# olsson-group/thermodynamic-interpolation

Measured on AMD Instinct MI355X. Metric: integration-steps/sec (whole node) + drift rel-L2 vs CPU ref, higher is better.
Workload: dtype f32 state and accumulation; matrix products on fp16 MFMA with 2-way split fp32 operands (hi + lo halves, 3 products)

## Files before the change

thermodynamic-interpolation_amd/csrc/painn_pair_kernel_body.inc:

```
{
    static_assert(PREC == 0 || PREC == 1, "the fp16 storage mode keeps the directed message kernel");
    constexpr int F = 16 * NBK, NB = (F + 31) / 32, T = 64 * WAVES, CH4 = edge_chunk4(NB, false);
    using A16 = r16::Act<NBK>;
    constexpr bool ONE = edge_one_chain(NB, PREC);
    using OP = std::conditional_t<ONE, r16::Opnd1<NBK>, typename r16::OpSel<NBK, PREC>::type>;
    extern __shared__ f32x4 lds[];
    const int lane = threadIdx.x & 63, wave = __builtin_amdgcn_readfirstlane(threadIdx.x >> 6), j = lane & 15, q = lane >> 4;
    constexpr int SC = pair_superchunk(), NBUF = pair_ring(WAVES);
    float* scratch = reinterpret_cast<float*>(lds + NBUF * SC * CH4) + wave * 64;
    float* vec = reinterpret_cast<float*>(lds + NBUF * SC * CH4) + WAVES * 64;
    for (int i = threadIdx.x; i < EV::COUNT * F / 4; i += T)
        reinterpret_cast<f32x4*>(vec)[i] = reinterpret_cast<const f32x4*>(p.vecs)[i];
#ifndef TI_PAIR_STAGGER
#define TI_PAIR_STAGGER 0
#endif
    PipeDMA<NB, T, SC, CH4, WAVES == 8 && TI_PAIR_STAGGER, NBUF> pipe;
    pipe.init(reinterpret_cast<const f32x4*>(p.stream), p.nch, lds, wave, lane);

    const float eps_w0 = ONE ? 1e-5f * p.wscale[0] * p.wscale[0] : 1e-5f, eps_w1 = ONE ? 1e-5f * p.wscale[1] * p.wscale[1] : 1e-5f;
    const float eps_p0 = ONE ? 1e-5f * p.wscale[2] * p.wscale[2] : 1e-5f, eps_p1 = ONE ? 1e-5f * p.wscale[3] * p.wscale[3] : 1e-5f;
    const float s_p0 = ONE ? p.wscale[2] : 1.0f, inv_out = ONE ? 1.0f / (p.wscale[4] * p.wscale[5]) : 1.0f;
    const long long gi_raw = (long long)blockIdx.x * WAVES + wave;
    const bool group_ok = gi_raw < p.n_groups;
    const long long gi = group_ok ? gi_raw : p.n_groups - 1;
    auto node_of = [&](int mol_local, int atom) {
        long long m = gi * p.G + mol_local;
        m = m < p.B ? m : p.B - 1;
        return m * p.A + atom;
    };

#ifdef TI_STAMPS
    constexpr int STAMP_SLOTS = 64;
    const bool st_wg = blockIdx.x >= 300 && blockIdx.x < 304;
    unsigned long long* const st_buf = p.stamps ? p.stamps + ((size_t)(blockIdx.x - 300) * WAVES + wave) * STAMP_SLOTS : nullptr;
    int st_i = 0;
    unsigned long long clk0 = 0, rt0 = 0;
    if (p.stamps) { clk0 = __builtin_amdgcn_s_memtime(); rt0 = __builtin_amdgcn_s_memrealtime(); }
#define TI_STAMP() do { if (st_wg && st_buf && blk == 3 && st_i < STAMP_SLOTS) { const unsigned long long t_ = __builtin_amdgcn_s_memtime(); if (lane == 0) st_buf[st_i] = t_; ++st_i; } } while (0)
#else
#define TI_STAMP() do { } while (0)
#endif

    for (int blk = 0; blk < p.nblk; ++blk) {
        TI_STAMP();
        const uint32_t meta = TI_PAIR_ROWS[blk * 16 + j];
        const long long nI = node_of(prow_molI(meta), prow_atomI(meta)), nJ = node_of(prow_molJ(meta), prow_atomJ(meta));
        const size_t brow0 = ((size_t)gi * p.nblk + blk) * 16;
        const size_t erowA = brow0 * 2, erowB = erowA + 16;
        OP enc;
        f32x4* const enc_park = reinterpret_cast<f32x4*>(p.enc) + (brow0 / 16) * (sizeof(OP) / 16) * 64 + lane;
        f32x4* const geo_park = reinterpret_cast<f32x4*>(p.geo) + brow0 + j;
        if constexpr (FIRST) {
            const float rx = p.x[nI * 3 + 0] - p.x[nJ * 3 + 0];
            const float ry = p.x[nI * 3 + 1] - p.x[nJ * 3 + 1];
            const float rz = p.x[nI * 3 + 2] - p.x[nJ * 3 + 2];
            const float dist = sqrtf(rx * rx + ry * ry + rz * rz);
            const float den = 1.0f + dist;
            if (q == 0) {
                f32x4 dd = {rx / den, ry / den, rz / den, 0.f};
                *reinterpret_cast<f32x4*>(scratch + j * 4) = dd;
                if (group_ok) *geo_park = dd;
            }
            A16 t;
            r16::posenc_set(t, dist / p.length_scale, q);
            enc.set(t);
            if (group_ok) r16::opnd_store(enc, enc_park);
        } else {
            if (q == 0) *reinterpret_cast<f32x4*>(scratch + j * 4) = *geo_park;
            r16::opnd_load(enc, enc_park);
        }
        TI_STAMP();
        OP g2;
        {
            OP g1;
            A16 t1;
#pragma unroll
            for (int c = 0; c < NB; ++c) {
                f32x4 a0 = r16::load_block(vec + EV::W_B0 * F, 2 * c, q), a1 = r16::load_block(vec + EV::W_B0 * F, 2 * c + 1, q);
                r16::gemm_on_pipe<false>(a0, a1, enc, pipe, lane);
                t1.b[2 * c] = a0; t1.b[2 * c + 1] = a1;
                pipe.release();
            }
            TI_STAMP();
            r16::ln_silu(t1, vec + EV::W_G0 * F, vec + EV::W_BE0 * F, q, eps_w0);
            g1.set(t1);
            TI_STAMP();
#pragma unroll
            for (int c = 0; c < NB; ++c) {
                f32x4 a0 = r16::load_block(vec + EV::W_B1 * F, 2 * c, q), a1 = r16::load_block(vec + EV::W_B1 * F, 2 * c + 1, q);
                r16::gemm_on_pipe<false>(a0, a1, g1, pipe, lane);
                t1.b[2 * c] = a0; t1.b[2 * c + 1] = a1;
                pipe.release();
            }
            TI_STAMP();
            r16::ln_silu(t1, vec + EV::W_G1 * F, vec + EV::W_BE1 * F, q, eps_w1);
            g2.set(t1);
            TI_STAMP();
        }
        OP h2A, h2B;
        {
            OP inA, inB;
            A16 tA, tB;
            float scA, scB;
            if (FIRST) {
                r16::load_set(tA, p.edge_emb + prow_type(meta) * F, q);
                scA = inA.set_scaled(tA);
                inB = inA; scB = scA;
            } else {
                r16::load_set(tA, p.e + (erowA + j) * F, q);
                r16::load_set(tB, p.e + (erowB + j) * F, q);
                scA = inA.set_scaled(tA);
                scB = inB.set_scaled(tB);
            }
            const float ivA = r16::pow2_inverse(scA) * s_p0, ivB = r16::pow2_inverse(scB) * s_p0;
            TI_STAMP();
#pragma unroll
            for (int c = 0; c < NB; ++c) {
                f32x4 a0 = r16::load_state<false>(p.P, (size_t)nI * F, 2 * c, q) * ivA, a1 = r16::load_state<false>(p.P, (size_t)nI * F, 2 * c + 1, q) * ivA;
                f32x4 b0 = r16::load_state<false>(p.P, (size_t)nJ * F, 2 * c, q) * ivB, b1 = r16::load_state<false>(p.P, (size_t)nJ * F, 2 * c + 1, q) * ivB;
                r16::gemm_x2_on_pipe<false>(a0, a1, b0, b1, inA, inB, pipe, lane);
                tA.b[2 * c] = a0 * scA; tA.b[2 * c + 1] = a1 * scA;
                tB.b[2 * c] = b0 * scB; tB.b[2 * c + 1] = b1 * scB;
                pipe.release();
            }
            TI_STAMP();
            r16::ln_silu(tA, vec + EV::P_G0 * F, vec + EV::P_BE0 * F, q, eps_p0);
            r16::ln_silu(tB, vec + EV::P_G0 * F, vec + EV::P_BE0 * F, q, eps_p0);
            inA.set(tA); inB.set(tB);
            TI_STAMP();
#pragma unroll
            for (int c = 0; c < NB; ++c) {
                f32x4 a0 = r16::load_block(vec + EV::P_B1 * F, 2 * c, q), a1 = r16::load_block(vec + EV::P_B1 * F, 2 * c + 1, q);
                f32x4 b0 = a0, b1 = a1;
                r16::gemm_x2_on_pipe<false>(a0, a1, b0, b1, inA, inB, pipe, lane);
                tA.b[2 * c] = a0; tA.b[2 * c + 1] = a1;
                tB.b[2 * c] = b0; tB.b[2 * c + 1] = b1;
                pipe.release();
            }
            TI_STAMP();
            r16::ln_silu(tA, vec + EV::P_G1 * F, vec + EV::P_BE1 * F, q, eps_p1);
            r16::ln_silu(tB, vec + EV::P_G1 * F, vec + EV::P_BE1 * F, q, eps_p1);
            h2A.set(tA); h2B.set(tB);
            TI_STAMP();
        }
        uint32_t mi[4];
#pragma unroll
        for (int r = 0; r < 4; ++r) mi[r] = TI_PAIR_ROWS[blk * 16 + 4 * q + r];
        f32x4 wfac;
#pragma unroll
        for (int r = 0; r < 4; ++r) wfac[r] = (mi[r] & 1u) ? inv_out : 0.0f;
#ifndef TI_PAIR_ACC_ATOMIC
#define TI_PAIR_ACC_ATOMIC 1
#endif
        float* const part_blk = p.part + ((size_t)gi * p.nblk + blk) * 8 * (7 * F);
        const int snJ = p.slotnode[blk * 16 + 4 + q], snI = p.slotnode[blk * 16 + q];
        const bool haveA = group_ok && snJ >= 0 && (!TI_PAIR_ACC_ATOMIC || gi * p.G + slot_mol(snJ) < p.B);
        const bool haveB = group_ok && snI >= 0 && (!TI_PAIR_ACC_ATOMIC || gi * p.G + slot_mol(snI) < p.B);
        float* const partA = part_blk + (size_t)(4 + q) * (7 * F);
        float* const partB = part_blk + (size_t)q * (7 * F);
        const int qnA = (int)((gi * p.G + slot_mol(snJ)) * p.A) + (snJ & 255), qnB = (int)((gi * p.G + slot_mol(snI)) * p.A) + (snI & 255);
        const bool qfA = (snJ & SLOT_FIRST_TOUCH) != 0, qfB = (snI & SLOT_FIRST_TOUCH) != 0;
        auto acc_ptr = [&](int node, int off) {
            return off < F ? p.dsacc + (size_t)node * F + off : off < 4 * F ? p.dvacc + (size_t)node * 3 * F + (off - F) : p.cacc + (size_t)node * 3 * F + (off - 4 * F);
        };
        const long long nIq = node_of(prow_molI(mi[0]), prow_atomI(mi[0]));

        auto out3 = [&](int c, int nbo, f32x4& rA0, f32x4& rA1, f32x4& rB0, f32x4& rB1) {
            f32x4 a0 = {0, 0, 0, 0}, a1 = {0, 0, 0, 0}, b0 = {0, 0, 0, 0}, b1 = {0, 0, 0, 0}, w0 = {0, 0, 0, 0}, w1 = {0, 0, 0, 0};
            r16::gemm_x2_on_pipe<true>(a0, a1, b0, b1, h2A, h2B, pipe, lane);
            pipe.release();
            r16::gemm_on_pipe<true>(w0, w1, g2, pipe, lane);
            pipe.release();
            const float* bp = vec + (EV::P_B2 + c) * F + 32 * nbo + j;
            const float* bw = vec + (EV::W_B2 + c) * F + 32 * nbo + j;
            w0 = (w0 + bw[0]) * wfac; w1 = (w1 + bw[16]) * wfac;
            rA0 = (a0 + bp[0]) * w0; rA1 = (a1 + bp[16]) * w1;
            rB0 = (b0 + bp[0]) * w0; rB1 = (b1 + bp[16]) * w1;
        };
        auto sumA = [&](const f32x4& v) {
            using QS = r16::QuarterSum<4>;
            return QS::swap32_add(QS::swap16_add(v[0], v[1]), QS::swap16_add(v[2], v[3]));
        };
        auto putA = [&](float z0, float z1, int off) {
            if (TI_PAIR_ACC_ATOMIC) { if (haveA) { float* d = acc_ptr(qnA, off); acc_out(d, z0, qfA); acc_out(d + 16, z1, qfA); } }
            else if (haveA) { partA[off] = z0; partA[off + 16] = z1; }
        };
        auto putB = [&](float z0, float z1, int off) {
            if (TI_PAIR_ACC_ATOMIC) { if (haveB) { float* d = acc_ptr(qnB, off); acc_out(d, z0, qfB); acc_out(d + 16, z1, qfB); } }
            else if (haveB) { partB[off] = z0; partB[off + 16] = z1; }
        };
        auto sumB = [&](const f32x4& v) { return (v[0] + v[1]) + (v[2] + v[3]); };
        auto emitA = [&](const f32x4& v0, const f32x4& v1, int off) { putA(sumA(v0), sumA(v1), off); };
        auto emitB = [&](const f32x4& v0, const f32x4& v1, int off) { putB(sumB(v0), sumB(v1), off); };
        auto rows4 = [&](float x, float (&o)[4]) {
            float a = x, b = x;
            lane_swap16(a, b);
            o[0] = a; o[2] = a; lane_swap32(o[0], o[2]);
            o[1] = b; o[3] = b; lane_swap32(o[1], o[3]);
        };
        constexpr bool GATHER_EARLY = PREC != 0;
        constexpr bool FOLD = pair_folds_cross(PREC) && !FIRST;
        f32x4* const zpark = reinterpret_cast<f32x4*>(vec + EV::COUNT * F) + wave * 3 * 64 + lane;
        static_assert(!FOLD || GATHER_EARLY, "the fold crosses with the v[dst] rows that the early gathers hold");
        const long long nJq = snJ >= 0 ? node_of(slot_mol(snJ), snJ & 255) : nIq;
        const float wrow = (meta & 1u) ? inv_out : 0.0f;

#pragma unroll 1
        for (int nbo = 0; nbo < NB; ++nbo) {
            const int fo = 32 * nbo + j;
            TI_STAMP();
            {
                f32x4 a0, a1, b0, b1;
                out3(2, nbo, a0, a1, b0, b1);
                emitA(a0, a1, fo);
                emitB(b0, b1, fo);
            }
            TI_STAMP();
            if constexpr (!LAST) {
                f32x4 a0 = r16::load_block(vec + (EV::P_B2 + 3) * F, 2 * nbo, q), a1 = r16::load_block(vec + (EV::P_B2 + 3) * F, 2 * nbo + 1, q);
                f32x4 b0 = a0, b1 = a1;
                f32x4 w0 = r16::load_block(vec + (EV::W_B2 + 3) * F, 2 * nbo, q), w1 = r16::load_block(vec + (EV::W_B2 + 3) * F, 2 * nbo + 1, q);
                float* const ea = p.e + (erowA + j) * F;
                float* const eb = p.e + (erowB + j) * F;
                f32x4 oA0, oA1, oB0, oB1;
                if (FIRST) {
                    const float* em = p.edge_emb + prow_type(meta) * F;
                    oA0 = r16::load_block(em, 2 * nbo, q); oA1 = r16::load_block(em, 2 * nbo + 1, q);
                    oB0 = oA0; oB1 = oA1;
                } else {
                    oA0 = r16::load_block(ea, 2 * nbo, q); oA1 = r16::load_block(ea, 2 * nbo + 1, q);
                    oB0 = r16::load_block(eb, 2 * nbo, q); oB1 = r16::load_block(eb, 2 * nbo + 1, q);
                }
                r16::gemm_x2_on_pipe<false>(a0, a1, b0, b1, h2A, h2B, pipe, lane);
                pipe.release();
                r16::gemm_on_pipe<false>(w0, w1, g2, pipe, lane);
                pipe.release();
                w0 *= wrow; w1 *= wrow;
                if (group_ok) {
                    r16::store_block(ea, 2 * nbo, q, oA0 + a0 * w0); r16::store_block(ea, 2 * nbo + 1, q, oA1 + a1 * w1);
                    r16::store_block(eb, 2 * nbo, q, oB0 + b0 * w0); r16::store_block(eb, 2 * nbo + 1, q, oB1 + b1 * w1);
                }
            }
            TI_STAMP();
            {
                f32x4 sA0, sA1, sB0, sB1, gA0 = {0, 0, 0, 0}, gA1 = {0, 0, 0, 0}, gB0 = {0, 0, 0, 0}, gB1 = {0, 0, 0, 0};
                out3(1, nbo, sA0, sA1, sB0, sB1);
                float vI[3][2], vJ[3][2];
                if (!FIRST) {
                    const float* vp = p.v + (size_t)nIq * 3 * F + fo;
                    const float* vq = p.v + (size_t)nJq * 3 * F + fo;
#pragma unroll
                    for (int c = 0; c < 3; ++c) {
                        vI[c][0] = vp[c * F]; vI[c][1] = vp[c * F + 16];
                        if (GATHER_EARLY) { vJ[c][0] = vq[c * F]; vJ[c][1] = vq[c * F + 16]; }
                    }
                    out3(0, nbo, gA0, gA1, gB0, gB1);
                }
                f32x4 dir[4];
#pragma unroll
                for (int r = 0; r < 4; ++r) dir[r] = *reinterpret_cast<const f32x4*>(scratch + (4 * q + r) * 4);
                float zA[3][2], zB[3][2];
#pragma unroll
                for (int c = 0; c < 3; ++c) {
                    f32x4 v0, v1;
#pragma unroll
                    for (int r = 0; r < 4; ++r) {
                        v0[r] = sA0[r] * dir[r][c]; v1[r] = sA1[r] * dir[r][c];
                        if (!FIRST) { v0[r] = fmaf(gA0[r], vI[c][0], v0[r]); v1[r] = fmaf(gA1[r], vI[c][1], v1[r]); }
                    }
                    zA[c][0] = sumA(v0); zA[c][1] = sumA(v1);
                    if (!GATHER_EARLY) putA(zA[c][0], zA[c][1], (1 + c) * F + fo);
                }
#pragma unroll
                for (int c = 0; c < 3; ++c) {
                    f32x4 v0, v1;
                    float j0[4], j1[4];
                    if (!FIRST) {
                        if (GATHER_EARLY) { rows4(vJ[c][0], j0); rows4(vJ[c][1], j1); }
                        else
#pragma unroll
                            for (int r = 0; r < 4; ++r) {
                                const float* vr = p.v + (size_t)node_of(prow_molJ(mi[r]), prow_atomJ(mi[r])) * 3 * F + c * F + fo;
                                j0[r] = vr[0]; j1[r] = vr[16];
                            }
                    }
#pragma unroll
                    for (int r = 0; r < 4; ++r) {
                        v0[r] = -(sB0[r] * dir[r][c]); v1[r] = -(sB1[r] * dir[r][c]);
                        if (!FIRST) { v0[r] = fmaf(gB0[r], j0[r], v0[r]); v1[r] = fmaf(gB1[r], j1[r], v1[r]); }
                    }
                    zB[c][0] = sumB(v0); zB[c][1] = sumB(v1);
                    if (!GATHER_EARLY) putB(zB[c][0], zB[c][1], (1 + c) * F + fo);
                }
                TI_STAMP();
                if constexpr (FOLD) {
                    zpark[0] = f32x4{zA[0][0], zA[0][1], zA[1][0], zA[1][1]};
                    zpark[64] = f32x4{zA[2][0], zA[2][1], zB[0][0], zB[0][1]};
                    zpark[128] = f32x4{zB[1][0], zB[1][1], zB[2][0], zB[2][1]};
                    f32x4 cA0, cA1, cB0, cB1;
                    out3(4, nbo, cA0, cA1, cB0, cB1);
                    f32x4 dc[4];
#pragma unroll
                    for (int r = 0; r < 4; ++r) dc[r] = *reinterpret_cast<const f32x4*>(scratch + (4 * q + r) * 4);
                    {
                        const f32x4 z0 = zpark[0], z1 = zpark[64], z2 = zpark[128];
                        zA[0][0] = z0[0]; zA[0][1] = z0[1]; zA[1][0] = z0[2]; zA[1][1] = z0[3];
                        zA[2][0] = z1[0]; zA[2][1] = z1[1]; zB[0][0] = z1[2]; zB[0][1] = z1[3];
                        zB[1][0] = z2[0]; zB[1][1] = z2[1]; zB[2][0] = z2[2]; zB[2][1] = z2[3];
                    }
                    float kA[3][2], kB[3][2];
#pragma unroll
                    for (int c = 0; c < 3; ++c) {
                        f32x4 a0, a1, b0, b1;
#pragma unroll
                        for (int r = 0; r < 4; ++r) {
                            a0[r] = cA0[r] * dc[r][c]; a1[r] = cA1[r] * dc[r][c];
                            b0[r] = -(cB0[r] * dc[r][c]); b1[r] = -(cB1[r] * dc[r][c]);
                        }
                        kA[c][0] = sumA(a0); kA[c][1] = sumA(a1);
                        kB[c][0] = sumB(b0); kB[c][1] = sumB(b1);
                    }
#pragma unroll
                    for (int c = 0; c < 3; ++c) {
                        const int c1 = (c + 1) % 3, c2 = (c + 2) % 3;
#pragma unroll
                        for (int h = 0; h < 2; ++h) {
                            zA[c][h] += kA[c1][h] * vJ[c2][h] - kA[c2][h] * vJ[c1][h];
                            zB[c][h] += kB[c1][h] * vI[c2][h] - kB[c2][h] * vI[c1][h];
                        }
                    }
                }
                if (GATHER_EARLY)
#pragma unroll
                    for (int c = 0; c < 3; ++c) { putA(zA[c][0], zA[c][1], (1 + c) * F + fo); putB(zB[c][0], zB[c][1], (1 + c) * F + fo); }
                if (!FIRST && !FOLD) {
                    f32x4 cA0, cA1, cB0, cB1;
                    out3(4, nbo, cA0, cA1, cB0, cB1);
#pragma unroll
                    for (int c = 0; c < 3; ++c) {
                        f32x4 v0, v1;
#pragma unroll
                        for (int r = 0; r < 4; ++r) { v0[r] = cA0[r] * dir[r][c]; v1[r] = cA1[r] * dir[r][c]; }
                        emitA(v0, v1, (4 + c) * F + fo);
                    }
#pragma unroll
                    for (int c = 0; c < 3; ++c) {
                        f32x4 v0, v1;
#pragma unroll
                        for (int r = 0; r < 4; ++r) { v0[r] = -(cB0[r] * dir[r][c]); v1[r] = -(cB1[r] * dir[r][c]); }
                        emitB(v0, v1, (4 + c) * F + fo);
                    }
                }
            }
        }
    }
    pipe.drain();
#ifdef TI_STAMPS
    if (p.stamps && lane == 0) {
        const unsigned long long clk1 = __builtin_amdgcn_s_memtime(), rt1 = __builtin_amdgcn_s_memrealtime();
        unsigned long long* c = p.stamps + 2048 + 2 * (size_t)gi_raw;
        c[0] = clk1 - clk0; c[1] = rt1 - rt0;
    }
#endif
}
```

thermodynamic-interpolation_amd/csrc/ti_api.hip:

```cpp
#include <algorithm>
#include <array>
#include <climits>
#include <cmath>
#include <cstdio>
#include <cstdlib>
#include <cstring>
#include <map>
#include <memory>
#include <stdexcept>
#include <utility>

#include "pair_template.hpp"
#include "ti_internal.hpp"

namespace ti {

static thread_local std::string g_err;
static int fail(int code, const std::string& msg) { g_err = msg; return code; }

struct HipError : std::runtime_error { using std::runtime_error::runtime_error; };
struct Unsupported : std::runtime_error { using std::runtime_error::runtime_error; };
#define HIP_CHECK(expr) do { hipError_t e__ = (expr); if (e__ != hipSuccess) \
    throw HipError(std::string(#expr) + ": " + hipGetErrorString(e__)); } while (0)

// ... 1617 lines not shown
        const float *xd = x, *cd = cond, *td = t; float *od = out, *dd = out_div;
        if (mem == TI_MEM_HOST) {
            if (h->rk_tv.n < (size_t)B) h->rk_tv.alloc(B);
            HIP_CHECK(hipMemcpyAsync(h->x.p, x, n * sizeof(float), hipMemcpyHostToDevice, h->stream));
            if (nc) HIP_CHECK(hipMemcpyAsync(h->cond.p, cond, nc * sizeof(float), hipMemcpyHostToDevice, h->stream));
            HIP_CHECK(hipMemcpyAsync(h->rk_tv.p, t, (size_t)B * sizeof(float), hipMemcpyHostToDevice, h->stream));
            xd = h->x.p; cd = h->cond.p; td = h->rk_tv.p; od = h->b1.p; dd = h->divb.p;
        }
        painn_drift_div_dev(h, xd, 0.f, cd, B, od, dd, td);
        if (mem == TI_MEM_HOST) {
            HIP_CHECK(hipMemcpyAsync(out, od, n * sizeof(float), hipMemcpyDeviceToHost, h->stream));
            HIP_CHECK(hipMemcpyAsync(out_div, dd, (size_t)B * sizeof(float), hipMemcpyDeviceToHost, h->stream));
        }
        HIP_CHECK(hipStreamSynchronize(h->stream));
        return TI_OK;
    });
}

static int painn_rollout_dlogp_impl(ti_handle* h, const ti_rollout_desc* rd, int n_probes, uint64_t probe_seed, const float* x0,
                                    const float* cond, int64_t B, float div_scale, float out_scale, int reverse_ode, float* out_path,
                                    float* out_dlogp, int64_t* n_fevals)
{
    if (!h || h->kind != 0) return fail(TI_E_ARG, "not a painn handle");
    if (h->d.precision == TI_PREC_F16) return fail(TI_E_UNSUPPORTED, "the fp16 storage mode has no divergence / tangent path (use f32 or f16x2)");
    if (int rc = check_rollout_desc(rd)) return rc;
    if (rd->scheme == TI_SCHEME_EM) return fail(TI_E_UNSUPPORTED, "dlogp is defined for the deterministic schemes only (EULER, HEUN)");
    if (rd->scheme == TI_SCHEME_DOPRI5_TRAJ && h->obs[1].K > 0)
        return fail(TI_E_UNSUPPORTED, "TI_SCHEME_DOPRI5_TRAJ writes its rows per trajectory inside a kernel: detach the observer (ti_obs_set_observer)");
    if (B < 0 || (B > 0 && (!x0 || !out_path || !out_dlogp || (h->ncond > 0 && !cond)))) return fail(TI_E_ARG, "NULL buffer");
    if (B == 0) { if (n_fevals) *n_fevals = 0; return TI_OK; }
    return guarded([&]() -> int {
        set_device(h);
        select_template(h, B, false);
        ensure_painn_ws(h, B);
        const int A = h->d.n_atoms;
        const size_t n = (size_t)B * A * 3, nc = (size_t)B * A * h->ncond;
        const hipMemcpyKind in_kind = rd->mem == TI_MEM_DEVICE ? hipMemcpyDeviceToDevice : hipMemcpyHostToDevice;
        HIP_CHECK(hipMemcpyAsync(h->x.p, x0, n * sizeof(float), in_kind, h->stream));
        const float* cd = cond;
        if (rd->mem == TI_MEM_HOST && nc) { HIP_CHECK(hipMemcpyAsync(h->cond.p, cond, nc * sizeof(float), hipMemcpyHostToDevice, h->stream)); cd = h->cond.p; }
        const int saved_tap = h->tap; h->tap = -1;
        const Ragged rg = ragged_of(h);
        if (n_probes > 0) painn_make_probes(h, B, n_probes, probe_seed, rd->traj_offset);
        DlogpAux aux;
        aux.dl = h->dl.p; aux.d1 = h->divb.p; aux.d2 = h->div2.p; aux.scaled = h->dlscaled.p; aux.out = out_dlogp;
        aux.n_dl = (size_t)B; aux.div_scale = div_scale; aux.out_scale = out_scale;
        auto drift = [&](const float* xs, float t, float* o, float* dv) {
            if (n_probes > 0) painn_drift_div_est_dev(h, xs, t, cd, B, n_probes, o, dv);
            else painn_drift_div_dev(h, xs, t, cd, B, o, dv);
            if (reverse_ode) {
                HIP_CHECK(launch_scale(o, o, -1.0f, (long long)n, h->stream));
                HIP_CHECK(launch_scale(dv, dv, -1.0f, (long long)B, h->stream));
            }
        };
        auto drift_tv = [&](const float* xs, const float* tv, float* o, float* dv) {
            if (n_probes > 0) painn_drift_div_est_dev(h, xs, 0.f, cd, B, n_probes, o, dv, tv);
            else painn_drift_div_dev(h, xs, 0.f, cd, B, o, dv, tv);
            if (reverse_ode) {
                HIP_CHECK(launch_scale(o, o, -1.0f, (long long)n, h->stream));
                HIP_CHECK(launch_scale(dv, dv, -1.0f, (long long)B, h->stream));
            }
        };
        const int rc = rd->scheme == TI_SCHEME_DOPRI5_TRAJ ? rollout_rk_traj(h, rd, h->x.p, B, A * 3, out_path, n_fevals, drift_tv, aux, rg)
                     : rd->scheme >= TI_SCHEME_DOPRI5 ? rollout_rk(h, rd, h->x.p, n, out_path, n_fevals, drift, aux, rg)
                                                      : rollout_common(h, rd, h->x.p, h->b1.p, h->b2.p, h->xt.p, n, B, A * 3, A, out_path, n_fevals, drift, aux, rg);
        h->tap = saved_tap;
        return rc;
    });
}

int ti_painn_rollout_dlogp(ti_handle* h, const ti_rollout_desc* rd, const float* x0, const float* cond, int64_t B, float div_scale,
                           float out_scale, int reverse_ode, float* out_path, float* out_dlogp, int64_t* n_fevals)
{
    return painn_rollout_dlogp_impl(h, rd, 0, 0, x0, cond, B, div_scale, out_scale, reverse_ode, out_path, out_dlogp, n_fevals);
}

int ti_painn_rollout_dlogp_est(ti_handle* h, const ti_rollout_desc* rd, int32_t n_probes, uint64_t probe_seed, const float* x0,
                               const float* cond, int64_t B, float div_scale, float out_scale, int reverse_ode, float* out_path,
                               float* out_dlogp, int64_t* n_fevals)
{
    if (!h || h->kind != 0) return fail(TI_E_ARG, "not a painn handle");
    if (h->d.precision == TI_PREC_F16) return fail(TI_E_UNSUPPORTED, "the fp16 storage mode has no divergence / tangent path (use f32 or f16x2)");
    if (n_probes < 1) return fail(TI_E_ARG, "n_probes must be >= 1");
    return painn_rollout_dlogp_impl(h, rd, n_probes, probe_seed, x0, cond, B, div_scale, out_scale, reverse_ode, out_path, out_dlogp, n_fevals);
}

static int painn_drift_div_est_impl(ti_handle* h, const float* x, float t, const float* tv, const float* cond, int64_t B, int32_t n_probes,
                                    uint64_t probe_seed, int64_t traj_offset, float* out, float* out_div, int mem, bool per_mol_t)
{
    if (!h || h->kind != 0) return fail(TI_E_ARG, "not a painn handle");
    if (h->d.precision == TI_PREC_F16) return fail(TI_E_UNSUPPORTED, "the fp16 storage mode has no divergence / tangent path (use f32 or f16x2)");
    if (n_probes < 1) return fail(TI_E_ARG, "n_probes must be >= 1");
    if (B < 0 || (B > 0 && (!x || (per_mol_t && !tv) || !out || !out_div || (h->ncond > 0 && !cond)))) return fail(TI_E_ARG, "NULL buffer");
    if (B == 0) return TI_OK;
    if (h->tap >= 0) return fail(TI_E_ARG, "debug taps apply to ti_painn_drift / ti_painn_drift_jvp only");
    return guarded([&]() -> int {
        set_device(h);
        select_template(h, B, false);
        ensure_painn_ws(h, B);
        const size_t n = (size_t)B * h->d.n_atoms * 3, nc = (size_t)B * h->d.n_atoms * h->ncond;
        const float *xd = x, *cd = cond, *td = tv; float *od = out, *dd = out_div;
        if (mem == TI_MEM_HOST) {
            HIP_CHECK(hipMemcpyAsync(h->x.p, x, n * sizeof(float), hipMemcpyHostToDevice, h->stream));
            if (nc) HIP_CHECK(hipMemcpyAsync(h->cond.p, cond, nc * sizeof(float), hipMemcpyHostToDevice, h->stream));
            if (per_mol_t) {
                if (h->rk_tv.n < (size_t)B) h->rk_tv.alloc(B);
                HIP_CHECK(hipMemcpyAsync(h->rk_tv.p, tv, (size_t)B * sizeof(float), hipMemcpyHostToDevice, h->stream));
                td = h->rk_tv.p;
            }
            xd = h->x.p; cd = h->cond.p; od = h->b1.p; dd = h->divb.p;
        }
        painn_make_probes(h, B, n_probes, probe_seed, traj_offset);
        painn_drift_div_est_dev(h, xd, t, cd, B, n_probes, od, dd, per_mol_t ? td : nullptr);
        if (mem == TI_MEM_HOST) {
            HIP_CHECK(hipMemcpyAsync(out, od, n * sizeof(float), hipMemcpyDeviceToHost, h->stream));
            HIP_CHECK(hipMemcpyAsync(out_div, dd, (size_t)B * sizeof(float), hipMemcpyDeviceToHost, h->stream));
        }
        HIP_CHECK(hipStreamSynchronize(h->stream));
        return TI_OK;
    });
}

int ti_painn_drift_div_est(ti_handle* h, const float* x, float t, const float* cond, int64_t B, int32_t n_probes, uint64_t probe_seed,
                           int64_t traj_offset, float* out, float* out_div, int mem)
{
    return painn_drift_div_est_impl(h, x, t, nullptr, cond, B, n_probes, probe_seed, traj_offset, out, out_div, mem, false);
}

int ti_painn_drift_div_est_tv(ti_handle* h, const float* x, const float* t, const float* cond, int64_t B, int32_t n_probes,
                              uint64_t probe_seed, int64_t traj_offset, float* out, float* out_div, int mem)
{
    return painn_drift_div_est_impl(h, x, 0.f, t, cond, B, n_probes, probe_seed, traj_offset, out, out_div, mem, true);
}

int ti_painn_debug_tap(ti_handle* h, int stage)
{
    if (!h || h->kind != 0) return fail(TI_E_ARG, "not a painn handle");
    if (h->d.precision == TI_PREC_F16 && stage >= 0) return fail(TI_E_UNSUPPORTED, "debug taps read fp32 state; not available in the fp16 storage mode");
    h->tap = stage;
    return TI_OK;
}

int ti_painn_debug_poison(ti_handle* h, int64_t B, float value)
{
    if (!h || h->kind != 0 || B <= 0) return fail(TI_E_ARG, "not a painn handle / B");
    return guarded([&]() -> int {
        set_device(h);
        ensure_painn_ws(h, B);
        const size_t N = (size_t)B * h->d.n_atoms, F = h->d.n_features;
        const unsigned bits = __builtin_bit_cast(unsigned, value);
        HIP_CHECK(hipMemsetD32Async((hipDeviceptr_t)h->dsacc.p, (int)bits, N * F, h->stream));
        HIP_CHECK(hipMemsetD32Async((hipDeviceptr_t)h->dvacc.p, (int)bits, N * 3 * F, h->stream));
        HIP_CHECK(hipMemsetD32Async((hipDeviceptr_t)h->cacc.p, (int)bits, N * 3 * F, h->stream));
        return TI_OK;
    });
}

int ti_painn_debug_read(ti_handle* h, int what, float* out, size_t n_floats)
{
    if (!h || h->kind != 0 || !out) return fail(TI_E_ARG, "bad argument");
    return guarded([&]() -> int {
        set_device(h);
        const size_t A = h->d.n_atoms, F = h->d.n_features, E = h->d.n_edges, B = (size_t)h->last_B, N = B * A;
        HIP_CHECK(hipStreamSynchronize(h->stream));
        if (what == 0) {
            if (n_floats != N * F) return fail(TI_E_ARG, "size mismatch (s)");
            std::vector<float> ds(n_floats);
            HIP_CHECK(hipMemcpy(out, h->s.p, n_floats * sizeof(float), hipMemcpyDeviceToHost));
            HIP_CHECK(hipMemcpy(ds.data(), h->dsacc.p, n_floats * sizeof(float), hipMemcpyDeviceToHost));
            for (size_t i = 0; i < n_floats; ++i) out[i] += ds[i];
        } else if (what == 1) {
            if (n_floats != N * 3 * F) return fail(TI_E_ARG, "size mismatch (v)");
            std::vector<float> v(n_floats), dv(n_floats), cc(n_floats);
            HIP_CHECK(hipMemcpy(v.data(), h->v.p, n_floats * sizeof(float), hipMemcpyDeviceToHost));
            HIP_CHECK(hipMemcpy(dv.data(), h->dvacc.p, n_floats * sizeof(float), hipMemcpyDeviceToHost));
            HIP_CHECK(hipMemcpy(cc.data(), h->cacc.p, n_floats * sizeof(float), hipMemcpyDeviceToHost));
            for (size_t nd = 0; nd < N; ++nd)
                for (size_t f = 0; f < F; ++f)
                    for (int c = 0; c < 3; ++c) {
                        const int c1 = (c + 1) % 3, c2 = (c + 2) % 3;
                        auto at = [&](const std::vector<float>& a, int cc2) { return a[(nd * 3 + cc2) * F + f]; };
                        out[(nd * 3 + c) * F + f] = (at(v, c) + at(dv, c)) + (at(cc, c1) * at(v, c2) - at(cc, c2) * at(v, c1));
                    }
        } else if (what == 2) {
            if (n_floats != B * E * F) return fail(TI_E_ARG, "size mismatch (e)");
            const size_t RB = ti::EDGE_ROWS_PER_BLOCK, rows = (B + h->G - 1) / h->G * h->parts * h->nblk * RB * (h->active == 2 ? 2 : 1);
            std::vector<float> e(rows * F);
            HIP_CHECK(hipMemcpy(e.data(), h->e.p, e.size() * sizeof(float), hipMemcpyDeviceToHost));
            for (size_t m = 0; m < B; ++m)
                for (size_t k = 0; k < E; ++k)
                    std::memcpy(out + (m * E + h->perm[k]) * F, e.data() + edge_row_of(h, m, k) * F, F * sizeof(float));
        } else if (what >= 3 && what <= 5) {
            if (h->last_D != 1 || (size_t)h->last_VB != B) return fail(TI_E_ARG, "tangent taps need a preceding ti_painn_drift_jvp call");
            auto fetch = [&](const DevBuf<float>& b, size_t n) { std::vector<float> v(n); HIP_CHECK(hipMemcpy(v.data(), b.p, n * sizeof(float), hipMemcpyDeviceToHost)); return v; };
            if (what == 3) {
                if (n_floats != N * F) return fail(TI_E_ARG, "size mismatch (ts)");
                const auto ts = fetch(h->ts, n_floats), td = fetch(h->tdsacc, n_floats);
                for (size_t i = 0; i < n_floats; ++i) out[i] = ts[i] + td[i];
            } else if (what == 4) {
                if (n_floats != N * 3 * F) return fail(TI_E_ARG, "size mismatch (tv)");
                const auto v = fetch(h->v, n_floats), cc = fetch(h->cacc, n_floats);
                const auto tv = fetch(h->tv, n_floats), tdv = fetch(h->tdvacc, n_floats), tcc = fetch(h->tcacc, n_floats);
                for (size_t nd = 0; nd < N; ++nd)
                    for (size_t f = 0; f < F; ++f)
                        for (int c = 0; c < 3; ++c) {
                            const int c1 = (c + 1) % 3, c2 = (c + 2) % 3;
                            auto at = [&](const std::vector<float>& a, int cc2) { return a[(nd * 3 + cc2) * F + f]; };
                            out[(nd * 3 + c) * F + f] = (at(tv, c) + at(tdv, c)) + ((at(tcc, c1) * at(v, c2) + at(cc, c1) * at(tv, c2)) -
                                                                                     (at(tcc, c2) * at(v, c1) + at(cc, c2) * at(tv, c1)));
                        }
            } else {
                if (n_floats != B * E * F) return fail(TI_E_ARG, "size mismatch (te)");
                const size_t RB = ti::EDGE_ROWS_PER_BLOCK, rows = (B + h->G - 1) / h->G * h->parts * h->nblk * RB;
                const auto e = fetch(h->te, rows * F);
                for (size_t m = 0; m < B; ++m)
                    for (size_t k = 0; k < E; ++k)
                        std::memcpy(out + (m * E + h->perm[k]) * F, e.data() + edge_row_of(h, m, k) * F, F * sizeof(float));
            }
        } else return fail(TI_E_ARG, "unknown tap");
        return TI_OK;
    });
}

ti_handle* ti_adw_create(const ti_adw_desc* d, const double* weights, size_t n_weights, int device)
{
    return ti_adw_create_nd(d, 1, weights, n_weights, device);
}

ti_handle* ti_adw_create_nd(const ti_adw_desc* d, int32_t dim, const double* weights, size_t n_weights, int device)
{
    ti_handle* out = nullptr;
    const int rc = guarded([&]() -> int {
        if (!d || !weights) return fail(TI_E_ARG, "NULL argument");
        if (dim < 1 || dim > 16) return fail(TI_E_UNSUPPORTED, "dim must be 1..16 (FCNetMultiBeta(d, d, H, L)), got " + std::to_string(dim));
        const int H = d->hidden_size, nl = d->num_layers;
        if (H != 32 && H != 64 && H != 128 && H != 256) return fail(TI_E_UNSUPPORTED, "hidden_size must be 32, 64, 128 or 256");
        if (nl < 1) return fail(TI_E_ARG, "num_layers must be >= 1");
        if (d->precision != TI_PREC_F32 && d->precision != TI_PREC_F16X2) return fail(TI_E_ARG, "unknown precision");
        const size_t need = (size_t)H * 3 + H + (size_t)H * H + H + H + 1 + (size_t)H * (dim + 2) + H + (size_t)(nl - 1) * ((size_t)H * H + H) +
                            (size_t)dim * H + dim;
        if (n_weights != need) return fail(TI_E_ARG, "weight count mismatch: expected " + std::to_string(need) + ", got " + std::to_string(n_weights));
        std::unique_ptr<ti_handle> h(new_handle(1, device));
        h->ad = *d; h->NB = H / 32; h->a_dim = dim;
        std::vector<float> w(n_weights);
        for (size_t i = 0; i < n_weights; ++i) w[i] = (float)weights[i];
        const int NB = h->NB, NBK = H / 16;
        const bool split = d->precision == TI_PREC_F16X2;
        std::vector<float> nat, pk;
        auto chunk16 = [&](const float* W, int row0) {
            if (split) pack_chunk16_split(pk, W, H, H, row0, 0, NBK); else pack_chunk16(pk, W, H, H, row0, 0, NBK);
        };
        auto take_mlp = [&](size_t& o, int n_hidden, size_t& vec_off, Stream& st, float& b_out, int D) {
            vec_off = nat.size();
            const int K = D + 2, Kpad = D == 1 ? 3 : (K + 3) / 4 * 4;
            for (int f = 0; f < H; ++f) {
                nat.insert(nat.end(), &w[o + (size_t)f * K], &w[o + (size_t)f * K] + K);
                nat.insert(nat.end(), (size_t)(Kpad - K), 0.f);
            }
            o += (size_t)H * K;
            nat.insert(nat.end(), &w[o], &w[o] + H); o += H;
            st.off4 = pk.size() / 4;
            std::vector<float> bh;
            for (int l = 0; l < n_hidden; ++l) {
                for (int nbo = 0; nbo < NB; ++nbo) chunk16(&w[o], 32 * nbo);
                o += (size_t)H * H;
                bh.insert(bh.end(), &w[o], &w[o] + H); o += H;
            }
            st.nch = n_hidden * NB;
            nat.insert(nat.end(), bh.begin(), bh.end());
            nat.insert(nat.end(), &w[o], &w[o] + (size_t)D * H); o += (size_t)D * H;
            if (D == 1) { b_out = w[o]; o += 1; return; }
            nat.insert(nat.end(), &w[o], &w[o] + D); o += D;
            nat.insert(nat.end(), (size_t)((D + 3) / 4 * 4 - D), 0.f);
            b_out = 0.f;
        };
        size_t o = 0;
        take_mlp(o, 1, h->a_be_vecs, h->st_be, h->a_be_b_out, 1);
        take_mlp(o, nl - 1, h->a_net_vecs, h->st_net, h->a_b_out, dim);
        if (pk.empty()) pk.assign(4, 0.f);
        h->flat.upload(nat); h->packed.upload(pk);
        HIP_CHECK(configure_adw_kernels(NB, std::max(1, nl - 1), dim));
        if (dim == 1) HIP_CHECK(configure_adw_fused_kernels(NB, std::max(1, nl - 1)));
        out = h.release();
        return TI_OK;
    });
    return rc == TI_OK ? out : nullptr;
}

static int adw_drift_impl(ti_handle* h, const float* x, float t, const float* beta0, const float* beta1, int64_t B, float* out,
                          float* out_div, int mem)
{
    if (!h || h->kind != 1) return fail(TI_E_ARG, "not an adw handle");
    if (B < 0 || (B > 0 && (!x || !beta0 || !beta1 || !out))) return fail(TI_E_ARG, "NULL buffer");
    if (B == 0) return TI_OK;
    return guarded([&]() -> int {
        set_device(h);
        ensure_adw_ws(h, B);
        const long long U = adw_set_cond(h, beta0, beta1, B, mem);
        const float* xd = x; float* od = out; float* dd = out_div;
        const size_t n = (size_t)B * h->a_dim;
        if (mem == TI_MEM_HOST) {
            HIP_CHECK(hipMemcpyAsync(h->ax.p, x, n * sizeof(float), hipMemcpyHostToDevice, h->stream));
            xd = h->ax.p; od = h->ab1.p; dd = out_div ? h->ad1.p : nullptr;
        }
        adw_drift_dev(h, xd, t, U, B, od, dd);
        if (mem == TI_MEM_HOST) {
// ... 505 lines not shown
```

Baseline: 475,100.

## Skip edge-state traffic for invalid pair rows, seed bias into MFMA, use group-base addressing

Invalid pair rows (meta bit 0 clear) no longer load or store the edge state, encoding park and geometry park. Their values are zero-filled in registers so the math stays defined. Node addressing moves to per-group base pointers with 32-bit local offsets, which replaces 64-bit index math. The output bias is seeded into the MFMA accumulator instead of being added afterwards. The debug poison fill now also covers the e/enc/geo buffers, so skipped rows can be checked. The risks are slightly different rounding from the seeded bias, and correctness now depends on invalid rows never being read downstream.

```diff
diff --git a/thermodynamic-interpolation_amd/csrc/painn_pair_kernel_body.inc b/thermodynamic-interpolation_amd/csrc/painn_pair_kernel_body.inc
--- a/thermodynamic-interpolation_amd/csrc/painn_pair_kernel_body.inc
+++ b/thermodynamic-interpolation_amd/csrc/painn_pair_kernel_body.inc
@@ -14,6 +14,15 @@
 #ifndef TI_PAIR_STAGGER
 #define TI_PAIR_STAGGER 0
 #endif
+#ifndef TI_PAIR_SEED_BIAS
+#define TI_PAIR_SEED_BIAS 1
+#endif
+#ifndef TI_PAIR_SKIP_INVALID
+#define TI_PAIR_SKIP_INVALID 1
+#endif
+#ifndef TI_PAIR_GROUP_BASE
+#define TI_PAIR_GROUP_BASE 1
+#endif
     PipeDMA<NB, T, SC, CH4, WAVES == 8 && TI_PAIR_STAGGER, NBUF> pipe;
     pipe.init(reinterpret_cast<const f32x4*>(p.stream), p.nch, lds, wave, lane);
 
@@ -28,6 +37,18 @@
         m = m < p.B ? m : p.B - 1;
         return m * p.A + atom;
     };
+    const long long gnode0 = gi * p.G * (long long)p.A;
+    const unsigned mol_cap = (unsigned)(p.B - 1 - gi * p.G);
+    auto lnode_of = [&](int mol_local, int atom) {
+        const unsigned m = (unsigned)mol_local < mol_cap ? (unsigned)mol_local : mol_cap;
+        return m * (unsigned)p.A + (unsigned)atom;
+    };
+    const float* const x_g = p.x + gnode0 * 3;
+    const float* const P_g = p.P + gnode0 * F;
+    const float* const v_g = p.v + gnode0 * 3 * F;
+    float* const ds_g = p.dsacc + gnode0 * F;
+    float* const dv_g = p.dvacc + gnode0 * 3 * F;
+    float* const c_g = p.cacc + gnode0 * 3 * F;
 
 #ifdef TI_STAMPS
     constexpr int STAMP_SLOTS = 64;
@@ -45,29 +66,38 @@
         TI_STAMP();
         const uint32_t meta = TI_PAIR_ROWS[blk * 16 + j];
         const long long nI = node_of(prow_molI(meta), prow_atomI(meta)), nJ = node_of(prow_molJ(meta), prow_atomJ(meta));
+        const unsigned lI = lnode_of(prow_molI(meta), prow_atomI(meta)), lJ = lnode_of(prow_molJ(meta), prow_atomJ(meta));
+        const bool row_ok = !TI_PAIR_SKIP_INVALID || (meta & 1u) != 0;
         const size_t brow0 = ((size_t)gi * p.nblk + blk) * 16;
         const size_t erowA = brow0 * 2, erowB = erowA + 16;
         OP enc;
         f32x4* const enc_park = reinterpret_cast<f32x4*>(p.enc) + (brow0 / 16) * (sizeof(OP) / 16) * 64 + lane;
         f32x4* const geo_park = reinterpret_cast<f32x4*>(p.geo) + brow0 + j;
         if constexpr (FIRST) {
-            const float rx = p.x[nI * 3 + 0] - p.x[nJ * 3 + 0];
-            const float ry = p.x[nI * 3 + 1] - p.x[nJ * 3 + 1];
-            const float rz = p.x[nI * 3 + 2] - p.x[nJ * 3 + 2];
+            const float* const xI = TI_PAIR_GROUP_BASE ? x_g + lI * 3u : p.x + nI * 3;
+            const float* const xJ = TI_PAIR_GROUP_BASE ? x_g + lJ * 3u : p.x + nJ * 3;
+            const float rx = xI[0] - xJ[0];
+            const float ry = xI[1] - xJ[1];
+            const float rz = xI[2] - xJ[2];
             const float dist = sqrtf(rx * rx + ry * ry + rz * rz);
             const float den = 1.0f + dist;
             if (q == 0) {
                 f32x4 dd = {rx / den, ry / den, rz / den, 0.f};
                 *reinterpret_cast<f32x4*>(scratch + j * 4) = dd;
-                if (group_ok) *geo_park = dd;
+                if (group_ok && row_ok) *geo_park = dd;
             }
             A16 t;
             r16::posenc_set(t, dist / p.length_scale, q);
             enc.set(t);
-            if (group_ok) r16::opnd_store(enc, enc_park);
+            if (group_ok && row_ok) r16::opnd_store(enc, enc_park);
         } else {
-            if (q == 0) *reinterpret_cast<f32x4*>(scratch + j * 4) = *geo_park;
-            r16::opnd_load(enc, enc_park);
+            if (q == 0) {
+                f32x4 dd = {0.f, 0.f, 0.f, 0.f};
+                if (row_ok) dd = *geo_park;
+                *reinterpret_cast<f32x4*>(scratch + j * 4) = dd;
+            }
+            if (TI_PAIR_SKIP_INVALID) __builtin_memset(&enc, 0, sizeof(OP));
+            if (row_ok) r16::opnd_load(enc, enc_park);
         }
         TI_STAMP();
         OP g2;
@@ -107,8 +137,14 @@
                 scA = inA.set_scaled(tA);
                 inB = inA; scB = scA;
             } else {
-                r16::load_set(tA, p.e + (erowA + j) * F, q);
-                r16::load_set(tB, p.e + (erowB + j) * F, q);
+                if (TI_PAIR_SKIP_INVALID) {
+#pragma unroll
+                    for (int nb = 0; nb < NBK; ++nb) { tA.b[nb] = f32x4{0.f, 0.f, 0.f, 0.f}; tB.b[nb] = f32x4{0.f, 0.f, 0.f, 0.f}; }
+                }
+                if (row_ok) {
+                    r16::load_set(tA, p.e + erowA * F + (unsigned)(j * F), q);
+                    r16::load_set(tB, p.e + erowB * F + (unsigned)(j * F), q);
+                }
                 scA = inA.set_scaled(tA);
                 scB = inB.set_scaled(tB);
             }
@@ -116,8 +152,10 @@
             TI_STAMP();
 #pragma unroll
             for (int c = 0; c < NB; ++c) {
-                f32x4 a0 = r16::load_state<false>(p.P, (size_t)nI * F, 2 * c, q) * ivA, a1 = r16::load_state<false>(p.P, (size_t)nI * F, 2 * c + 1, q) * ivA;
-                f32x4 b0 = r16::load_state<false>(p.P, (size_t)nJ * F, 2 * c, q) * ivB, b1 = r16::load_state<false>(p.P, (size_t)nJ * F, 2 * c + 1, q) * ivB;
+                const float* const PI = TI_PAIR_GROUP_BASE ? P_g + lI * (unsigned)F : p.P + (size_t)nI * F;
+                const float* const PJ = TI_PAIR_GROUP_BASE ? P_g + lJ * (unsigned)F : p.P + (size_t)nJ * F;
+                f32x4 a0 = r16::load_block(PI, 2 * c, q) * ivA, a1 = r16::load_block(PI, 2 * c + 1, q) * ivA;
+                f32x4 b0 = r16::load_block(PJ, 2 * c, q) * ivB, b1 = r16::load_block(PJ, 2 * c + 1, q) * ivB;
                 r16::gemm_x2_on_pipe<false>(a0, a1, b0, b1, inA, inB, pipe, lane);
                 tA.b[2 * c] = a0 * scA; tA.b[2 * c + 1] = a1 * scA;
                 tB.b[2 * c] = b0 * scB; tB.b[2 * c + 1] = b1 * scB;
@@ -160,33 +198,49 @@
         float* const partB = part_blk + (size_t)q * (7 * F);
         const int qnA = (int)((gi * p.G + slot_mol(snJ)) * p.A) + (snJ & 255), qnB = (int)((gi * p.G + slot_mol(snI)) * p.A) + (snI & 255);
         const bool qfA = (snJ & SLOT_FIRST_TOUCH) != 0, qfB = (snI & SLOT_FIRST_TOUCH) != 0;
-        auto acc_ptr = [&](int node, int off) {
+        const unsigned lnA = (unsigned)slot_mol(snJ) * (unsigned)p.A + (unsigned)(snJ & 255), lnB = (unsigned)slot_mol(snI) * (unsigned)p.A + (unsigned)(snI & 255);
+        auto acc_ptr = [&](int node, unsigned lnode, int off) {
+            if (TI_PAIR_GROUP_BASE)
+                return off < F ? ds_g + (lnode * (unsigned)F + (unsigned)off) : off < 4 * F ? dv_g + (lnode * (unsigned)(3 * F) + (unsigned)(off - F)) : c_g + (lnode * (unsigned)(3 * F) + (unsigned)(off - 4 * F));
             return off < F ? p.dsacc + (size_t)node * F + off : off < 4 * F ? p.dvacc + (size_t)node * 3 * F + (off - F) : p.cacc + (size_t)node * 3 * F + (off - 4 * F);
         };
         const long long nIq = node_of(prow_molI(mi[0]), prow_atomI(mi[0]));
+        const unsigned lIq = lnode_of(prow_molI(mi[0]), prow_atomI(mi[0]));
 
         auto out3 = [&](int c, int nbo, f32x4& rA0, f32x4& rA1, f32x4& rB0, f32x4& rB1) {
-            f32x4 a0 = {0, 0, 0, 0}, a1 = {0, 0, 0, 0}, b0 = {0, 0, 0, 0}, b1 = {0, 0, 0, 0}, w0 = {0, 0, 0, 0}, w1 = {0, 0, 0, 0};
-            r16::gemm_x2_on_pipe<true>(a0, a1, b0, b1, h2A, h2B, pipe, lane);
-            pipe.release();
-            r16::gemm_on_pipe<true>(w0, w1, g2, pipe, lane);
-            pipe.release();
             const float* bp = vec + (EV::P_B2 + c) * F + 32 * nbo + j;
             const float* bw = vec + (EV::W_B2 + c) * F + 32 * nbo + j;
-            w0 = (w0 + bw[0]) * wfac; w1 = (w1 + bw[16]) * wfac;
-            rA0 = (a0 + bp[0]) * w0; rA1 = (a1 + bp[16]) * w1;
-            rB0 = (b0 + bp[0]) * w0; rB1 = (b1 + bp[16]) * w1;
+            if (TI_PAIR_SEED_BIAS) {
+                const float p0 = bp[0], p1 = bp[16], q0 = bw[0], q1 = bw[16];
+                f32x4 a0 = {p0, p0, p0, p0}, a1 = {p1, p1, p1, p1}, b0 = a0, b1 = a1, w0 = {q0, q0, q0, q0}, w1 = {q1, q1, q1, q1};
+                r16::gemm_x2_on_pipe<true>(a0, a1, b0, b1, h2A, h2B, pipe, lane);
+                pipe.release();
+                r16::gemm_on_pipe<true>(w0, w1, g2, pipe, lane);
+                pipe.release();
+                w0 *= wfac; w1 *= wfac;
+                rA0 = a0 * w0; rA1 = a1 * w1;
+                rB0 = b0 * w0; rB1 = b1 * w1;
+            } else {
+                f32x4 a0 = {0, 0, 0, 0}, a1 = {0, 0, 0, 0}, b0 = {0, 0, 0, 0}, b1 = {0, 0, 0, 0}, w0 = {0, 0, 0, 0}, w1 = {0, 0, 0, 0};
+                r16::gemm_x2_on_pipe<true>(a0, a1, b0, b1, h2A, h2B, pipe, lane);
+                pipe.release();
+                r16::gemm_on_pipe<true>(w0, w1, g2, pipe, lane);
+                pipe.release();
+                w0 = (w0 + bw[0]) * wfac; w1 = (w1 + bw[16]) * wfac;
+                rA0 = (a0 + bp[0]) * w0; rA1 = (a1 + bp[16]) * w1;
+                rB0 = (b0 + bp[0]) * w0; rB1 = (b1 + bp[16]) * w1;
+            }
         };
         auto sumA = [&](const f32x4& v) {
             using QS = r16::QuarterSum<4>;
             return QS::swap32_add(QS::swap16_add(v[0], v[1]), QS::swap16_add(v[2], v[3]));
         };
         auto putA = [&](float z0, float z1, int off) {
-            if (TI_PAIR_ACC_ATOMIC) { if (haveA) { float* d = acc_ptr(qnA, off); acc_out(d, z0, qfA); acc_out(d + 16, z1, qfA); } }
+            if (TI_PAIR_ACC_ATOMIC) { if (haveA) { float* d = acc_ptr(qnA, lnA, off); acc_out(d, z0, qfA); acc_out(d + 16, z1, qfA); } }
             else if (haveA) { partA[off] = z0; partA[off + 16] = z1; }
         };
         auto putB = [&](float z0, float z1, int off) {
-            if (TI_PAIR_ACC_ATOMIC) { if (haveB) { float* d = acc_ptr(qnB, off); acc_out(d, z0, qfB); acc_out(d + 16, z1, qfB); } }
+            if (TI_PAIR_ACC_ATOMIC) { if (haveB) { float* d = acc_ptr(qnB, lnB, off); acc_out(d, z0, qfB); acc_out(d + 16, z1, qfB); } }
             else if (haveB) { partB[off] = z0; partB[off + 16] = z1; }
         };
         auto sumB = [&](const f32x4& v) { return (v[0] + v[1]) + (v[2] + v[3]); };
@@ -203,6 +257,7 @@
         f32x4* const zpark = reinterpret_cast<f32x4*>(vec + EV::COUNT * F) + wave * 3 * 64 + lane;
         static_assert(!FOLD || GATHER_EARLY, "the fold crosses with the v[dst] rows that the early gathers hold");
         const long long nJq = snJ >= 0 ? node_of(slot_mol(snJ), snJ & 255) : nIq;
+        const unsigned lJq = snJ >= 0 ? lnode_of(slot_mol(snJ), snJ & 255) : lIq;
         const float wrow = (meta & 1u) ? inv_out : 0.0f;
 
 #pragma unroll 1
@@ -220,23 +275,26 @@
                 f32x4 a0 = r16::load_block(vec + (EV::P_B2 + 3) * F, 2 * nbo, q), a1 = r16::load_block(vec + (EV::P_B2 + 3) * F, 2 * nbo + 1, q);
                 f32x4 b0 = a0, b1 = a1;
                 f32x4 w0 = r16::load_block(vec + (EV::W_B2 + 3) * F, 2 * nbo, q), w1 = r16::load_block(vec + (EV::W_B2 + 3) * F, 2 * nbo + 1, q);
-                float* const ea = p.e + (erowA + j) * F;
-                float* const eb = p.e + (erowB + j) * F;
+                float* const ea = p.e + erowA * F + (unsigned)(j * F);
+                float* const eb = p.e + erowB * F + (unsigned)(j * F);
                 f32x4 oA0, oA1, oB0, oB1;
                 if (FIRST) {
                     const float* em = p.edge_emb + prow_type(meta) * F;
                     oA0 = r16::load_block(em, 2 * nbo, q); oA1 = r16::load_block(em, 2 * nbo + 1, q);
                     oB0 = oA0; oB1 = oA1;
                 } else {
-                    oA0 = r16::load_block(ea, 2 * nbo, q); oA1 = r16::load_block(ea, 2 * nbo + 1, q);
-                    oB0 = r16::load_block(eb, 2 * nbo, q); oB1 = r16::load_block(eb, 2 * nbo + 1, q);
+                    if (TI_PAIR_SKIP_INVALID) oA0 = oA1 = oB0 = oB1 = f32x4{0.f, 0.f, 0.f, 0.f};
+                    if (row_ok) {
+                        oA0 = r16::load_block(ea, 2 * nbo, q); oA1 = r16::load_block(ea, 2 * nbo + 1, q);
+                        oB0 = r16::load_block(eb, 2 * nbo, q); oB1 = r16::load_block(eb, 2 * nbo + 1, q);
+                    }
                 }
                 r16::gemm_x2_on_pipe<false>(a0, a1, b0, b1, h2A, h2B, pipe, lane);
                 pipe.release();
                 r16::gemm_on_pipe<false>(w0, w1, g2, pipe, lane);
                 pipe.release();
                 w0 *= wrow; w1 *= wrow;
-                if (group_ok) {
+                if (group_ok && row_ok) {
                     r16::store_block(ea, 2 * nbo, q, oA0 + a0 * w0); r16::store_block(ea, 2 * nbo + 1, q, oA1 + a1 * w1);
                     r16::store_block(eb, 2 * nbo, q, oB0 + b0 * w0); r16::store_block(eb, 2 * nbo + 1, q, oB1 + b1 * w1);
                 }
@@ -247,8 +305,8 @@
                 out3(1, nbo, sA0, sA1, sB0, sB1);
                 float vI[3][2], vJ[3][2];
                 if (!FIRST) {
-                    const float* vp = p.v + (size_t)nIq * 3 * F + fo;
-                    const float* vq = p.v + (size_t)nJq * 3 * F + fo;
+                    const float* vp = TI_PAIR_GROUP_BASE ? v_g + (lIq * (unsigned)(3 * F) + (unsigned)fo) : p.v + (size_t)nIq * 3 * F + fo;
+                    const float* vq = TI_PAIR_GROUP_BASE ? v_g + (lJq * (unsigned)(3 * F) + (unsigned)fo) : p.v + (size_t)nJq * 3 * F + fo;
 #pragma unroll
                     for (int c = 0; c < 3; ++c) {
                         vI[c][0] = vp[c * F]; vI[c][1] = vp[c * F + 16];
@@ -280,7 +338,8 @@
                         else
 #pragma unroll
                             for (int r = 0; r < 4; ++r) {
-                                const float* vr = p.v + (size_t)node_of(prow_molJ(mi[r]), prow_atomJ(mi[r])) * 3 * F + c * F + fo;
+                                const float* vr = TI_PAIR_GROUP_BASE ? v_g + (lnode_of(prow_molJ(mi[r]), prow_atomJ(mi[r])) * (unsigned)(3 * F) + (unsigned)(c * F + fo))
+                                                                     : p.v + (size_t)node_of(prow_molJ(mi[r]), prow_atomJ(mi[r])) * 3 * F + c * F + fo;
                                 j0[r] = vr[0]; j1[r] = vr[16];
                             }
                     }
diff --git a/thermodynamic-interpolation_amd/csrc/ti_api.hip b/thermodynamic-interpolation_amd/csrc/ti_api.hip
--- a/thermodynamic-interpolation_amd/csrc/ti_api.hip
+++ b/thermodynamic-interpolation_amd/csrc/ti_api.hip
@@ -1793,6 +1793,10 @@
         HIP_CHECK(hipMemsetD32Async((hipDeviceptr_t)h->dsacc.p, (int)bits, N * F, h->stream));
         HIP_CHECK(hipMemsetD32Async((hipDeviceptr_t)h->dvacc.p, (int)bits, N * 3 * F, h->stream));
         HIP_CHECK(hipMemsetD32Async((hipDeviceptr_t)h->cacc.p, (int)bits, N * 3 * F, h->stream));
+        static_assert(sizeof(*h->e.p) == 4 && sizeof(*h->enc.p) == 4 && sizeof(*h->geo.p) == 4, "32-bit fills");
+        HIP_CHECK(hipMemsetD32Async((hipDeviceptr_t)h->e.p, (int)bits, h->e.n, h->stream));
+        HIP_CHECK(hipMemsetD32Async((hipDeviceptr_t)h->enc.p, (int)bits, h->enc.n, h->stream));
+        HIP_CHECK(hipMemsetD32Async((hipDeviceptr_t)h->geo.p, (int)bits, h->geo.n, h->stream));
         return TI_OK;
     });
 }
```

Result: faster. 483,900, median of 6 (+1.8%).
